# AOADMM-DataFusionFramework/Matlab-Code

Hardware: AMD Instinct MI355X
Metric: AO-ADMM outer iters/sec (+ mode-1 MTTKRP GFLOP/s), 2000^3 rank-20 CP (higher is better)
Workload: dtype f32

## Files before the change

matlab-code_amd/csrc/contract.hip:

```cpp
#include "contract.h"
#include "device_utils.h"
#include "small_dev.h"

#include <algorithm>
#include <cstdlib>

namespace aoadmm {

typedef float f32x4 __attribute__((ext_vector_type(4)));
typedef double f64x2 __attribute__((ext_vector_type(2)));
typedef double f64x4 __attribute__((ext_vector_type(4)));

static constexpr int kTileRows = 128;
static constexpr int kGroup = 8;

struct KArgs {
  const void* X;
  const void* frag;
  void* T;
  int64_t tiles_per_batch, ntiles, batch_stride, M, ld, C, Cg, trows;
  int groups_per_chunk, R;
  int flush_every;
};

// ... 661 lines not shown
  int groups_per_chunk, R;
  float inv_s;
};

template <int NT>
__global__ __launch_bounds__(256, NT <= 2 ? 2 : 1) void contract16_f16(KArgs16 a) {
  const int lane = threadIdx.x & 63;
  const int64_t wt = (int64_t)blockIdx.x * 4 + (threadIdx.x >> 6);
  if (wt >= a.ntiles) return;
  const int chunk = blockIdx.y;
  const int64_t blk = wt >> 2;
  const int m0 = (int)(wt & 3) * kTileRows;
  const int r16 = lane & 15, q = lane >> 4;
  const int64_t g0 = (int64_t)chunk * a.groups_per_chunk;
  int64_t g1 = g0 + a.groups_per_chunk;
  if (g1 > a.Cg) g1 = a.Cg;
  const int64_t ng = g1 > g0 ? g1 - g0 : 0;
  const _Float16* xp = a.X + (blk * a.Cg + g0) * kGroupHalves + (m0 + r16) * kGroup16 + 8 * q;
  const f16x8* fp = reinterpret_cast<const f16x8*>(reinterpret_cast<const char*>(a.frag) + kFragHeader16) + g0 * (NT * 128) + lane;

  f32x4 acc[NT][8];
#pragma unroll
  for (int nt = 0; nt < NT; ++nt)
#pragma unroll
    for (int t = 0; t < 8; ++t) acc[nt][t] = f32x4{0.f, 0.f, 0.f, 0.f};

  f16x8 x0[8], x1[8], x2[8];
  f16x8 f0[NT][2], f1[NT][2], f2[NT][2];
#define AO_LOAD1(XS, GI, TL) XS[TL] = __builtin_nontemporal_load(reinterpret_cast<const f16x8*>(xp + (GI) * kGroupHalves + (TL) * (16 * kGroup16)));
#define AO_LOADF(FS, GI)                                                                             \
  {                                                                                                  \
    _Pragma("unroll") for (int nt = 0; nt < NT; ++nt) {                                              \
      FS[nt][0] = fp[(GI) * (NT * 128) + nt * 128];                                                  \
      FS[nt][1] = fp[(GI) * (NT * 128) + nt * 128 + 64];                                             \
    }                                                                                                \
  }
#define AO_LOAD_STAGE(XS, FS, GI)                                                                    \
  { _Pragma("unroll") for (int tl_ = 0; tl_ < 8; ++tl_) AO_LOAD1(XS, GI, tl_) AO_LOADF(FS, GI) }
#define AO_FMA_T(XS, FS, TL)                                                                         \
  {                                                                                                  \
    _Pragma("unroll") for (int nt = 0; nt < NT; ++nt) {                                              \
      acc[nt][TL] = __builtin_amdgcn_mfma_f32_16x16x32_f16(XS[TL], FS[nt][0], acc[nt][TL], 0, 0, 0); \
      acc[nt][TL] = __builtin_amdgcn_mfma_f32_16x16x32_f16(XS[TL], FS[nt][1], acc[nt][TL], 0, 0, 0); \
    }                                                                                                \
  }
#define AO_COMPUTE_STAGE(XS, FS) { _Pragma("unroll") for (int tl_ = 0; tl_ < 8; ++tl_) AO_FMA_T(XS, FS, tl_) }
#define AO_MIX_STAGE(XC, FC, XL, FL, GI)                                                             \
  {                                                                                                  \
    _Pragma("unroll") for (int tl_ = 0; tl_ < 8; ++tl_) {                                            \
      AO_FMA_T(XC, FC, tl_) AO_LOAD1(XL, GI, tl_)                                                    \
      if (tl_ == 7) AO_LOADF(FL, GI)                                                                 \
      __builtin_amdgcn_sched_barrier(0);                                                             \
    }                                                                                                \
  }
  if (ng > 0) AO_LOAD_STAGE(x0, f0, 0)
  if (ng > 1) AO_LOAD_STAGE(x1, f1, 1)
  int64_t g = 0;
  for (; g + 5 <= ng; g += 3) {
    AO_MIX_STAGE(x0, f0, x2, f2, g + 2)
    AO_MIX_STAGE(x1, f1, x0, f0, g + 3)
    AO_MIX_STAGE(x2, f2, x1, f1, g + 4)
  }
  for (; g + 3 <= ng; g += 3) {
    if (g + 2 < ng) AO_LOAD_STAGE(x2, f2, g + 2)
    AO_COMPUTE_STAGE(x0, f0)
    if (g + 3 < ng) AO_LOAD_STAGE(x0, f0, g + 3)
    AO_COMPUTE_STAGE(x1, f1)
    if (g + 4 < ng) AO_LOAD_STAGE(x1, f1, g + 4)
    AO_COMPUTE_STAGE(x2, f2)
  }
  if (g < ng) AO_COMPUTE_STAGE(x0, f0)
  if (g + 1 < ng) AO_COMPUTE_STAGE(x1, f1)
#undef AO_LOAD1
#undef AO_LOADF
#undef AO_LOAD_STAGE
#undef AO_FMA_T
#undef AO_COMPUTE_STAGE
#undef AO_MIX_STAGE
  extern __shared__ __attribute__((aligned(16))) float t_lds[];
  float* tl = t_lds + (threadIdx.x >> 6) * (kTileRows * a.R);
  const float* tinv = reinterpret_cast<const float*>(reinterpret_cast<const char*>(a.frag) + 512);
#pragma unroll
  for (int nt = 0; nt < NT; ++nt) {
    const int r = 16 * nt + r16;
    if (r < a.R) {
      const float ti = tinv[r];
#pragma unroll
      for (int t = 0; t < 8; ++t)
#pragma unroll
        for (int i = 0; i < 4; ++i) tl[(16 * t + 4 * q + i) * a.R + r] = acc[nt][t][i] * ti * a.inv_s;
    }
  }
  {
    const int n16 = kTileRows * a.R / 4;
    f32x4* dst = reinterpret_cast<f32x4*>(a.T + ((int64_t)chunk * a.trows + blk * 512 + m0) * a.R);
    const f32x4* src = reinterpret_cast<const f32x4*>(tl);
    for (int c = lane; c < n16; c += 64) __builtin_nontemporal_store(src[c], dst + c);
  }
}

static int nt_of(int R, int prec) {
  const int w = prec == AOADMM_PREC_F32 ? 32 : 16;
  return (R + w - 1) / w;
}
static int tile_rows(int prec) { return prec == AOADMM_PREC_F64 ? kTileRows64 : kTileRows; }

size_t ContractPlan::frag_bytes(int prec) const {
  if (prec == AOADMM_PREC_F16)
    return (size_t)kFragHeader16 + (size_t)cdiv(C, kGroup16) * nt_of(R, prec) * 2048;
  const int64_t Cg = cdiv(C, kGroup);
  return (size_t)(nt_of(R, prec) * 1024 + 1152) * Cg + 8192;
}

ContractPlan make_plan(int64_t nbatch, int64_t batch_stride, int64_t M, int64_t ld, int64_t C, int R,
                       int prec) {
  ContractPlan p;
  const bool half = prec == AOADMM_PREC_F16;
  p.tprec = half ? AOADMM_PREC_F32 : prec;
  p.nbatch = nbatch; p.batch_stride = batch_stride; p.M = M; p.ld = ld; p.C = C; p.R = R;
  const int gcols = half ? kGroup16 : kGroup;
  const int64_t Cg = cdiv(C, gcols);
  const int64_t ntiles = nbatch * cdiv(M, tile_rows(prec));
  int64_t nchunk = 1;
  if (prec != AOADMM_PREC_F64) nchunk = cdiv(Cg, 2048 / gcols);
  if (ntiles < 2048) {
    int64_t want = cdiv(2048, ntiles);
    const int64_t gmin = 128 / gcols;
    int64_t maxc = Cg / gmin > 0 ? Cg / gmin : 1;
    if (want > maxc) want = maxc;
    if (want > nchunk) nchunk = want;
  }
  if (nchunk > 65535) nchunk = 65535;
  p.nchunk = (int)nchunk;
  return p;
}

ContractPlan make_lead_plan(int64_t M, int64_t ld, int64_t C, int R) {
  ContractPlan p;
  p.tprec = AOADMM_PREC_F32;
  p.nbatch = 1; p.batch_stride = 0; p.M = M; p.ld = ld; p.C = C; p.R = R;
  p.lead = true;
  const int64_t nch = cdiv(C, kLeadKC);
  p.nchunk = (int)cdiv(nch, 2048 / kLeadKC);
  return p;
}

static void launch_contract_lead(const void* X, const ContractPlan& pl, const double* F, int64_t ldF, void* frag_ws,
                                 void* T, hipStream_t s, hipEvent_t ev0, hipEvent_t ev1) {
  const int64_t Cg = cdiv(pl.C, kGroup);
  AO_REQUIRE(pl.ld % 4 == 0 && pl.ld >= 4, "f32 layout must be padded to 4");
  LArgs a;
  a.X = (const float*)X; a.frag = (const float*)frag_ws; a.T = (float*)T;
  a.M = pl.M; a.ld = pl.ld; a.C = pl.C; a.Cg = Cg; a.R = pl.R;
  a.chunks_per_slice = (int)cdiv(cdiv(pl.C, kLeadKC), pl.nchunk);
  const int64_t nblk = cdiv(pl.M, kLeadRows);
  AO_REQUIRE(nblk < (int64_t)2147483647, "tensor too large for one launch");
  dim3 grid((unsigned)nblk, (unsigned)pl.nchunk);
  const size_t sh = (size_t)2 * kLeadRows * kLeadStride * sizeof(float);
  const int nt16 = (pl.R + 15) / 16;
  const int64_t Cg16 = cdiv(pl.C, 16) + 1;
  const int64_t total = (int64_t)nt16 * Cg16 * 256;
  pack_frag_lead16_f32<<<(unsigned)cdiv(total, 256), 256, 0, s>>>(F, ldF, pl.C, pl.R, nt16, Cg16, (float*)frag_ws);
  AO_KERNEL_CHECK();
#define AO_SET(K) ensure_dynamic_lds(reinterpret_cast<const void*>(K), (int)sh);
  if (nt16 == 1) AO_SET(contract_lead16_f32<1>)
  else if (nt16 == 2) AO_SET(contract_lead16_f32<2>)
  else if (nt16 == 3) AO_SET(contract_lead16_f32<3>)
  else if (nt16 == 4) AO_SET(contract_lead16_f32<4>)
#undef AO_SET
  if (ev0) AO_HIP(hipEventRecord(ev0, s));
  if (nt16 == 1) contract_lead16_f32<1><<<grid, 256, sh, s>>>(a);
  else if (nt16 == 2) contract_lead16_f32<2><<<grid, 256, sh, s>>>(a);
  else if (nt16 == 3) contract_lead16_f32<3><<<grid, 256, sh, s>>>(a);
  else if (nt16 == 4) contract_lead16_f32<4><<<grid, 256, sh, s>>>(a);
  else throw Error(AOADMM_ERR_UNSUPPORTED, "rank > 64 not supported");
  if (ev1) AO_HIP(hipEventRecord(ev1, s));
  AO_KERNEL_CHECK();
}

static void launch_contract_half(const void* X, const ContractPlan& pl, const double* F, int64_t ldF, void* frag_ws,
                                 void* T, hipStream_t s, hipEvent_t ev0, hipEvent_t ev1) {
  AO_REQUIRE(pl.on_copy && !pl.lead && pl.M == 512 && pl.ld == 512 && pl.tprec == AOADMM_PREC_F32,
             "internal: a half operand is streamed from its pass copies only");
  const int64_t Cg = cdiv(pl.C, kGroup16);
  AO_REQUIRE(pl.batch_stride == 512 * kGroup16 * Cg && pl.nbatch > 0 && pl.C > 0, "internal: half pass copy and plan disagree");
  const int NT = nt_of(pl.R, AOADMM_PREC_F16);
  char* ws = reinterpret_cast<char*>(frag_ws);
  double* tsc = reinterpret_cast<double*>(ws);
  float* tinv = reinterpret_cast<float*>(ws + 512);
  frag16_scales_k<<<(unsigned)pl.R, 256, 0, s>>>(F, ldF, pl.C, tsc, tinv);
  AO_KERNEL_CHECK();
  pack_frag16_f16<<<(unsigned)cdiv(Cg * NT * 128, 256), 256, 0, s>>>(F, ldF, pl.C, pl.R, NT, Cg, tsc,
                                                                    reinterpret_cast<f16x8*>(ws + kFragHeader16));
  AO_KERNEL_CHECK();
  KArgs16 a;
  a.X = reinterpret_cast<const _Float16*>(X); a.frag = frag_ws; a.T = reinterpret_cast<float*>(T);
  a.ntiles = pl.nbatch * 4; a.Cg = Cg; a.trows = pl.trows();
  a.groups_per_chunk = (int)cdiv(Cg, pl.nchunk);
  a.R = pl.R;
  a.inv_s = (float)(1.0 / pl.xscale);
  AO_REQUIRE(pl.nbatch < (int64_t)2147483647, "tensor too large for one launch");
  const dim3 grid((unsigned)pl.nbatch, (unsigned)pl.nchunk);
  const size_t tsh = (size_t)4 * kTileRows * pl.R * sizeof(float);
#define AO_GO(K) { if (tsh > 65536) ensure_dynamic_lds(reinterpret_cast<const void*>(K), (int)tsh); if (ev0) AO_HIP(hipEventRecord(ev0, s)); K<<<grid, 256, tsh, s>>>(a); }
  if (NT == 1) AO_GO(contract16_f16<1>)
  else if (NT == 2) AO_GO(contract16_f16<2>)
  else if (NT == 3) AO_GO(contract16_f16<3>)
  else if (NT == 4) AO_GO(contract16_f16<4>)
  else throw Error(AOADMM_ERR_UNSUPPORTED, "rank > 64 not supported");
#undef AO_GO
  if (ev1) AO_HIP(hipEventRecord(ev1, s));
  AO_KERNEL_CHECK();
}

void launch_contract(const void* X, int prec, const ContractPlan& pl, const double* F, int64_t ldF,
                     void* frag_ws, void* T, hipStream_t s, hipEvent_t ev0, hipEvent_t ev1) {
  AO_REQUIRE(pl.R >= 1 && pl.R <= kMaxRank, "rank %d outside [1,%d]", pl.R, kMaxRank);
  if (prec == AOADMM_PREC_F16) {
    launch_contract_half(X, pl, F, ldF, frag_ws, T, s, ev0, ev1);
    return;
  }
  AO_REQUIRE(prec == AOADMM_PREC_F32 || prec == AOADMM_PREC_F64, "bad precision id %d", prec);
  AO_REQUIRE(pl.tprec == prec, "contraction plan and tensor precision disagree");
  if (pl.lead) {
    AO_REQUIRE(prec == AOADMM_PREC_F32, "leading-mode contraction exists for fp32 tensors only");
    launch_contract_lead(X, pl, F, ldF, frag_ws, T, s, ev0, ev1);
    return;
  }
  const int64_t Cg = cdiv(pl.C, kGroup);
  KArgs a;
  a.X = X; a.frag = frag_ws; a.T = T;
  a.tiles_per_batch = cdiv(pl.M, tile_rows(prec));
  a.ntiles = pl.nbatch * a.tiles_per_batch;
  a.batch_stride = pl.batch_stride; a.M = pl.M; a.ld = pl.ld; a.C = pl.C; a.Cg = Cg;
  a.trows = pl.trows();
  a.groups_per_chunk = (int)cdiv(Cg, pl.nchunk);
  a.R = pl.R;
  AO_REQUIRE(a.ntiles > 0 && pl.C > 0, "empty contraction");
  dim3 grid((unsigned)cdiv(a.ntiles, 4), (unsigned)pl.nchunk);
  AO_REQUIRE(cdiv(a.ntiles, 4) < (int64_t)2147483647, "tensor too large for one launch");
  if (prec == AOADMM_PREC_F32) {
    AO_REQUIRE(pl.ld % 4 == 0 && pl.M % 4 == 0 && pl.batch_stride % 4 == 0, "f32 layout must be padded to 4");
    const int rem = pl.R % 16;
    const bool ex = pl.R > 16 && rem >= 1 && rem <= 4;
    const int nt16 = ex ? pl.R / 16 : (pl.R + 15) / 16;
    const int64_t total = (int64_t)nt16 * Cg * 128 + (ex ? Cg * 32 : 0);
    pack_frag16_f32<<<(unsigned)cdiv(total, 256), 256, 0, s>>>(F, ldF, pl.C, pl.R, nt16, ex ? 1 : 0, Cg, (float*)frag_ws);
    AO_KERNEL_CHECK();
    size_t tsh = (size_t)4 * kTileRows * pl.R * sizeof(float);
    a.flush_every = kFlushEvery;
    if (nt16 == 1) tsh = (size_t)4 * 16384;
#define AO_GO(K) { if (tsh > 65536) ensure_dynamic_lds(reinterpret_cast<const void*>(K), (int)tsh); if (ev0) AO_HIP(hipEventRecord(ev0, s)); K<<<grid, 256, tsh, s>>>(a); }
    if (nt16 == 1 && !ex) AO_GO((contract16_f32<1, false, true>))
    else if (nt16 == 1) AO_GO((contract16_f32<1, true, true>))
    else if (nt16 == 2 && !ex) AO_GO((contract16_f32<2, false>))
    else if (nt16 == 2) AO_GO((contract16_f32<2, true>))
    else if (nt16 == 3 && !ex) AO_GO((contract16_f32<3, false>))
    else if (nt16 == 3) AO_GO((contract16_f32<3, true>))
    else if (nt16 == 4) AO_GO((contract16_f32<4, false>))
    else throw Error(AOADMM_ERR_UNSUPPORTED, "rank > 64 not supported");
#undef AO_GO
  } else {
    AO_REQUIRE(pl.ld % 2 == 0 && pl.M % 2 == 0 && pl.batch_stride % 2 == 0, "f64 layout must be padded to 2");
    const int rem = pl.R % 16;
    const bool ex = pl.R > 16 && rem >= 1 && rem <= 4;
    const int nt16 = ex ? pl.R / 16 : (pl.R + 15) / 16;
    const int64_t total = (int64_t)nt16 * Cg * 128 + (ex ? Cg * 32 : 0);
    pack_frag_f64<<<(unsigned)cdiv(total, 256), 256, 0, s>>>(F, ldF, pl.C, pl.R, nt16, ex ? 1 : 0, Cg, (double*)frag_ws);
    AO_KERNEL_CHECK();
    const size_t tsh = (size_t)4 * kTileRows64 * pl.R * sizeof(double);
#define AO_GO(K) { if (tsh > 65536) ensure_dynamic_lds(reinterpret_cast<const void*>(K), (int)tsh); if (ev0) AO_HIP(hipEventRecord(ev0, s)); K<<<grid, 256, tsh, s>>>(a); }
    if (nt16 == 1 && !ex) AO_GO((contract_f64<1, false>))
    else if (nt16 == 1) AO_GO((contract_f64<1, true>))
    else if (nt16 == 2 && !ex) AO_GO((contract_f64<2, false>))
    else if (nt16 == 2) AO_GO((contract_f64<2, true>))
    else if (nt16 == 3 && !ex) AO_GO((contract_f64<3, false>))
    else if (nt16 == 3) AO_GO((contract_f64<3, true>))
    else if (nt16 == 4) AO_GO((contract_f64<4, false>))
    else throw Error(AOADMM_ERR_UNSUPPORTED, "rank > 64 not supported");
#undef AO_GO
  }
  if (ev1) AO_HIP(hipEventRecord(ev1, s));
  AO_KERNEL_CHECK();
}

__global__ void factor_rowmajor_k(const double* __restrict__ F, int64_t ldF, int64_t rows, int R,
                                  double* __restrict__ Ft) {
  const int64_t idx = (int64_t)blockIdx.x * blockDim.x + threadIdx.x;
  if (idx >= rows * R) return;
  const int r = (int)(idx / rows);
  const int64_t a = idx - (int64_t)r * rows;
  Ft[a * R + r] = F[a + ldF * r];
}
static void factor_rowmajor(const double* F, int64_t ldF, int64_t rows, int R, double* Ft, hipStream_t s) {
  factor_rowmajor_k<<<(unsigned)cdiv(rows * R, 256), 256, 0, s>>>(F, ldF, rows, R, Ft);
  AO_KERNEL_CHECK();
}

template <typename TT, int VEC> struct TVec;
template <> struct TVec<float, 4> { typedef float type __attribute__((ext_vector_type(4))); };
template <> struct TVec<float, 1> { typedef float type; };
template <> struct TVec<double, 2> { typedef double type __attribute__((ext_vector_type(2))); };
template <> struct TVec<double, 1> { typedef double type; };
template <typename TT, int VEC>
__device__ __forceinline__ void fma_vec(double (&acc)[VEC], const TT* __restrict__ tp, const double* __restrict__ fp) {
  typedef typename TVec<TT, VEC>::type V;
  const V tv = __builtin_nontemporal_load(reinterpret_cast<const V*>(tp));
  if constexpr (VEC == 1) {
    acc[0] += (double)tv * fp[0];
  } else {
#pragma unroll
    for (int v = 0; v < VEC; ++v) acc[v] += (double)tv[v] * fp[v];
  }
}

template <typename TT, int VEC>
struct RVec {
  typename TVec<TT, VEC>::type t;
  double f[VEC];
  __device__ __forceinline__ void load(const TT* __restrict__ tp, const double* __restrict__ fp) {
    t = __builtin_nontemporal_load(reinterpret_cast<const typename TVec<TT, VEC>::type*>(tp));
#pragma unroll
    for (int v = 0; v < VEC; ++v) f[v] = fp[v];
  }
  __device__ __forceinline__ void fma(double (&acc)[VEC]) const {
    if constexpr (VEC == 1) {
      acc[0] += (double)t * f[0];
    } else {
#pragma unroll
      for (int v = 0; v < VEC; ++v) acc[v] += (double)t[v] * f[v];
    }
  }
};

template <typename TT, int VEC>
__global__ void reduce_inner_k(const TT* __restrict__ T, int nchunk, int64_t trows, int64_t A, int64_t Apad, int R,
                               const double* __restrict__ FaT, double scale, double* __restrict__ out,
                               int64_t ldOut, int rowmajor, int has_sys, SysBuild sys) {
  extern __shared__ double sh[];
  if (has_sys && blockIdx.x == 0) { sys_build_rider(sys); return; }
  const int64_t b = (int64_t)blockIdx.x - has_sys;
  const int t = threadIdx.x;
  const int64_t n = A * R, step = (int64_t)blockDim.x * VEC;
  double s0[VEC], s1[VEC], s2[VEC], s3[VEC];
#pragma unroll
  for (int v = 0; v < VEC; ++v) { s0[v] = 0; s1[v] = 0; s2[v] = 0; s3[v] = 0; }
  for (int ch = 0; ch < nchunk; ++ch) {
    const TT* Tb = T + ((int64_t)ch * trows + Apad * b) * R;
    int64_t e = (int64_t)t * VEC;
    for (; e + 3 * step < n; e += 4 * step) {
      RVec<TT, VEC> q0, q1, q2, q3;
      q0.load(Tb + e, FaT + e);
      q1.load(Tb + e + step, FaT + e + step);
      q2.load(Tb + e + 2 * step, FaT + e + 2 * step);
      q3.load(Tb + e + 3 * step, FaT + e + 3 * step);
      __builtin_amdgcn_sched_barrier(0);
      q0.fma(s0); q1.fma(s1); q2.fma(s2); q3.fma(s3);
    }
    for (; e < n; e += step) fma_vec<TT, VEC>(s0, Tb + e, FaT + e);
  }
#pragma unroll
  for (int v = 0; v < VEC; ++v) sh[t * VEC + v] = (s0[v] + s1[v]) + (s2[v] + s3[v]);
  __syncthreads();
  if (t < R) {
    const int nA = blockDim.x * VEC / R;
    double tot = 0.0;
    for (int i = 0; i < nA; ++i) tot += sh[i * R + t];
    if (rowmajor) out[b * R + t] = scale * tot;
    else out[b + ldOut * t] = scale * tot;
  }
}

template <typename TT, int VEC>
__global__ void reduce_inner2_k(const TT* __restrict__ T, int nchunk, int64_t trows, int64_t A, int64_t Apad, int64_t B,
                                int R, const double* __restrict__ FaT, double scale, double* __restrict__ out,
                                int64_t ldOut, int rowmajor, int has_sys, SysBuild sys) {
  extern __shared__ double sh[];
  if (has_sys && blockIdx.x == 0) { sys_build_rider(sys); return; }
  const int64_t b0 = 2 * ((int64_t)blockIdx.x - has_sys);
  const bool two = b0 + 1 < B;
  const int64_t b1 = two ? b0 + 1 : b0;
  const int t = threadIdx.x;
  const int64_t n = A * R, step = (int64_t)blockDim.x * VEC;
  double a0[VEC], a1[VEC], c0[VEC], c1[VEC];
#pragma unroll
  for (int v = 0; v < VEC; ++v) { a0[v] = 0; a1[v] = 0; c0[v] = 0; c1[v] = 0; }
  for (int ch = 0; ch < nchunk; ++ch) {
    const TT* Ta = T + ((int64_t)ch * trows + Apad * b0) * R;
    const TT* Tc = T + ((int64_t)ch * trows + Apad * b1) * R;
    int64_t e = (int64_t)t * VEC;
    for (; e + step < n; e += 2 * step) {
      RVec<TT, VEC> q0, q1, p0, p1;
      q0.load(Ta + e, FaT + e);
      q1.load(Ta + e + step, FaT + e + step);
      p0.t = __builtin_nontemporal_load(reinterpret_cast<const typename TVec<TT, VEC>::type*>(Tc + e));
      p1.t = __builtin_nontemporal_load(reinterpret_cast<const typename TVec<TT, VEC>::type*>(Tc + e + step));
      __builtin_amdgcn_sched_barrier(0);
#pragma unroll
      for (int v = 0; v < VEC; ++v) { p0.f[v] = q0.f[v]; p1.f[v] = q1.f[v]; }
      q0.fma(a0); q1.fma(a1); p0.fma(c0); p1.fma(c1);
    }
    for (; e < n; e += step) {
      RVec<TT, VEC> q0, p0;
      q0.load(Ta + e, FaT + e);
      p0.t = __builtin_nontemporal_load(reinterpret_cast<const typename TVec<TT, VEC>::type*>(Tc + e));
#pragma unroll
      for (int v = 0; v < VEC; ++v) p0.f[v] = q0.f[v];
      q0.fma(a0); p0.fma(c0);
    }
  }
  const int nt = blockDim.x * VEC;
#pragma unroll
  for (int v = 0; v < VEC; ++v) { sh[t * VEC + v] = a0[v] + a1[v]; sh[nt + t * VEC + v] = c0[v] + c1[v]; }
  __syncthreads();
  if (t < 2 * R) {
    const int which = t / R, r = t % R;
    if (which == 0 || two) {
      const int nA = nt / R;
      double tot = 0.0;
      for (int i = 0; i < nA; ++i) tot += sh[which * nt + i * R + r];
      const int64_t b = which ? b1 : b0;
      if (rowmajor) out[b * R + r] = scale * tot;
      else out[b + ldOut * r] = scale * tot;
    }
  }
}

size_t reduce_factor_scratch_bytes(int64_t rows, int R) { return (size_t)rows * R * sizeof(double); }

template <typename TT, int VEC>
static void launch_inner_t(const void* T, int nchunk, int64_t trows, int64_t A, int64_t Apad, int64_t B, int R,
                           const double* FaT, double scale, double* out, int64_t ldOut, hipStream_t s, int rowmajor,
                           const SysBuild* sys) {
  const int hs = sys ? 1 : 0;
  const SysBuild sb = sys ? *sys : SysBuild();
  const int rq = R / VEC;
  int threads = 256 / rq * rq;
  if (threads < rq) threads = rq;
  if (threads * VEC < R) threads = (R + VEC - 1) / VEC;
  if (B >= 1024 && 2 * R <= threads) {
    reduce_inner2_k<TT, VEC><<<(unsigned)((B + 1) / 2 + hs), threads, (size_t)2 * threads * VEC * sizeof(double), s>>>(
        (const TT*)T, nchunk, trows, A, Apad, B, R, FaT, scale, out, ldOut, rowmajor, hs, sb);
    return;
  }
  reduce_inner_k<TT, VEC><<<(unsigned)(B + hs), threads, (size_t)threads * VEC * sizeof(double), s>>>(
      (const TT*)T, nchunk, trows, A, Apad, R, FaT, scale, out, ldOut, rowmajor, hs, sb);
}

static bool sys_can_ride(const SysBuild* sys, int threads_min = 64) {
  return sys != nullptr && sys->R >= 1 && sys->R <= kSysRiderMaxR && threads_min >= 64;
}

bool launch_reduce_inner(const void* T, int tprec, int nchunk, int64_t trows, int64_t A, int64_t Apad,
                         int64_t B, int R, const double* Fa, int64_t ldFa, double scale,
                         double* out, int64_t ldOut, double* ft_scratch, hipStream_t s, const double* FaT,
                         int rowmajor_out, const SysBuild* sys) {
  AO_REQUIRE((int64_t)B < 2147483647ll, "reduce_inner: too many output rows for one launch");
  {
    const int vec = tprec == AOADMM_PREC_F32 ? (R % 4 == 0 ? 4 : 1) : (R % 2 == 0 ? 2 : 1);
    const int rq = R / vec;
    int threads = 256 / rq * rq;
    if (threads < rq) threads = rq;
    if (threads * vec < R) threads = (R + vec - 1) / vec;
    if (!sys_can_ride(sys, threads)) sys = nullptr;
  }
  if (FaT) ft_scratch = const_cast<double*>(FaT);
  else factor_rowmajor(Fa, ldFa, A, R, ft_scratch, s);
  if (tprec == AOADMM_PREC_F32) {
    if (R % 4 == 0) launch_inner_t<float, 4>(T, nchunk, trows, A, Apad, B, R, ft_scratch, scale, out, ldOut, s, rowmajor_out, sys);
    else launch_inner_t<float, 1>(T, nchunk, trows, A, Apad, B, R, ft_scratch, scale, out, ldOut, s, rowmajor_out, sys);
  } else {
    if (R % 2 == 0) launch_inner_t<double, 2>(T, nchunk, trows, A, Apad, B, R, ft_scratch, scale, out, ldOut, s, rowmajor_out, sys);
    else launch_inner_t<double, 1>(T, nchunk, trows, A, Apad, B, R, ft_scratch, scale, out, ldOut, s, rowmajor_out, sys);
  }
  AO_KERNEL_CHECK();
  return sys != nullptr;
}

static void outer_geometry(int64_t A, int64_t B, int R, int vec, int& TA, int64_t& nblkA, int& SB) {
  const int rq = (R + vec - 1) / vec;
  TA = 256 / rq;
  if (TA < 1) TA = 1;
  nblkA = cdiv(A, TA);
  int64_t sb = cdiv(2048, nblkA);
  if (sb > 64) sb = 64;
  if (sb > B) sb = B;
  if (sb < 1) sb = 1;
  SB = (int)sb;
}
static int outer_vec(int tprec, int R) {
  if (tprec == AOADMM_PREC_F32) return R % 4 == 0 ? 4 : 1;
  return R % 2 == 0 ? 2 : 1;
}

size_t reduce_outer_scratch_bytes(int64_t A, int64_t B, int R) {
  size_t worst = 0;
  for (int vec : {1, 2, 4}) {
    int TA, SB; int64_t nb;
    outer_geometry(A, B, R, vec, TA, nb, SB);
    worst = std::max(worst, (size_t)SB * A * R * sizeof(double));
  }
  return worst;
}

template <typename TT, int VEC>
__global__ void reduce_outer_k(const TT* __restrict__ T, int nchunk, int64_t trows, int64_t A,
                               int64_t Apad, int64_t B, int R, int TA, const double* __restrict__ FbT,
                               double* __restrict__ part, int has_sys, SysBuild sys) {
  if (has_sys && blockIdx.x == 0) {
    if (blockIdx.y == 0) sys_build_rider(sys);
    return;
  }
  const int t = threadIdx.x;
  const int rq = R / VEC;
  const int al = t / rq, r = (t - al * rq) * VEC;
  const int64_t a = ((int64_t)blockIdx.x - has_sys) * TA + al;
  const int SB = gridDim.y, sb = blockIdx.y;
  const int64_t bper = (B + SB - 1) / SB;
  const int64_t b0 = sb * bper;
  int64_t b1 = b0 + bper;
  if (b1 > B) b1 = B;
  if (al >= TA || a >= A) return;
  const int64_t bs = Apad * R;
  double s0[VEC], s1[VEC], s2[VEC], s3[VEC];
#pragma unroll
  for (int v = 0; v < VEC; ++v) { s0[v] = 0; s1[v] = 0; s2[v] = 0; s3[v] = 0; }
  for (int ch = 0; ch < nchunk; ++ch) {
    const TT* Tc = T + (int64_t)ch * trows * R + a * R + r;
    const double* Fr = FbT + r;
    int64_t b = b0;
    for (; b + 3 < b1; b += 4) {
      RVec<TT, VEC> q0, q1, q2, q3;
      q0.load(Tc + bs * b, Fr + b * R);
      q1.load(Tc + bs * (b + 1), Fr + (b + 1) * R);
      q2.load(Tc + bs * (b + 2), Fr + (b + 2) * R);
      q3.load(Tc + bs * (b + 3), Fr + (b + 3) * R);
      __builtin_amdgcn_sched_barrier(0);
      q0.fma(s0); q1.fma(s1); q2.fma(s2); q3.fma(s3);
    }
    for (; b < b1; ++b) fma_vec<TT, VEC>(s0, Tc + bs * b, Fr + b * R);
  }
#pragma unroll
  for (int v = 0; v < VEC; ++v) part[((int64_t)sb * A + a) * R + r + v] = (s0[v] + s1[v]) + (s2[v] + s3[v]);
}

__global__ void reduce_outer_fin(const double* __restrict__ part, int SB, int64_t A, int R, double scale,
                                 double* __restrict__ out, int64_t ldOut, int rowmajor) {
  int64_t idx = (int64_t)blockIdx.x * blockDim.x + threadIdx.x;
  if (idx >= A * R) return;
  const int64_t a = idx / R;
  const int r = (int)(idx - a * R);
  double t0 = 0.0, t1 = 0.0;
  int s = 0;
  const int64_t ar = A * R;
  for (; s + 7 < SB; s += 8) {
    const double v0 = part[(int64_t)s * ar + idx], v1 = part[(int64_t)(s + 1) * ar + idx];
    const double v2 = part[(int64_t)(s + 2) * ar + idx], v3 = part[(int64_t)(s + 3) * ar + idx];
    const double v4 = part[(int64_t)(s + 4) * ar + idx], v5 = part[(int64_t)(s + 5) * ar + idx];
    const double v6 = part[(int64_t)(s + 6) * ar + idx], v7 = part[(int64_t)(s + 7) * ar + idx];
    t0 += v0; t1 += v1; t0 += v2; t1 += v3; t0 += v4; t1 += v5; t0 += v6; t1 += v7;
  }
  for (; s + 1 < SB; s += 2) {
    t0 += part[(int64_t)s * ar + idx];
    t1 += part[(int64_t)(s + 1) * ar + idx];
  }
  if (s < SB) t0 += part[(int64_t)s * ar + idx];
  if (rowmajor) out[idx] = scale * (t0 + t1);
  else out[a + ldOut * r] = scale * (t0 + t1);
}

template <typename TT, int VEC>
static void launch_outer_t(const void* T, int nchunk, int64_t trows, int64_t A, int64_t Apad, int64_t B, int R,
                           const double* FbT, double* scratch, int& SB, hipStream_t s, const SysBuild* sys) {
  int TA; int64_t nb;
  outer_geometry(A, B, R, VEC, TA, nb, SB);
  int threads = TA * (R / VEC);
  threads = (threads + 63) / 64 * 64;
  const int hs = sys ? 1 : 0;
  reduce_outer_k<TT, VEC><<<dim3((unsigned)(nb + hs), (unsigned)SB), threads, 0, s>>>((const TT*)T, nchunk, trows, A, Apad, B,
                                                                                    R, TA, FbT, scratch, hs, sys ? *sys : SysBuild());
}

bool launch_reduce_outer(const void* T, int tprec, int nchunk, int64_t trows, int64_t A, int64_t Apad,
                         int64_t B, int R, const double* Fb, int64_t ldFb, double scale,
                         double* out, int64_t ldOut, double* scratch, double* ft_scratch, hipStream_t s,
                         const double* FbT, int rowmajor_out, const SysBuild* sys) {
  if (!sys_can_ride(sys)) sys = nullptr;
  if (FbT) ft_scratch = const_cast<double*>(FbT);
  else factor_rowmajor(Fb, ldFb, B, R, ft_scratch, s);
  int SB = 1;
  const int vec = outer_vec(tprec, R);
  if (tprec == AOADMM_PREC_F32) {
    if (vec == 4) launch_outer_t<float, 4>(T, nchunk, trows, A, Apad, B, R, ft_scratch, scratch, SB, s, sys);
    else launch_outer_t<float, 1>(T, nchunk, trows, A, Apad, B, R, ft_scratch, scratch, SB, s, sys);
  } else {
    if (vec == 2) launch_outer_t<double, 2>(T, nchunk, trows, A, Apad, B, R, ft_scratch, scratch, SB, s, sys);
    else launch_outer_t<double, 1>(T, nchunk, trows, A, Apad, B, R, ft_scratch, scratch, SB, s, sys);
  }
  AO_KERNEL_CHECK();
  reduce_outer_fin<<<(unsigned)cdiv(A * R, 256), 256, 0, s>>>(scratch, SB, A, R, scale, out, ldOut, rowmajor_out);
  AO_KERNEL_CHECK();
  return sys != nullptr;
}

template <typename TT, int RMAX>
__global__ __launch_bounds__(256) void small_mttkrp_k(SmallMttkrp a, int has_sys, SysBuild sys) {
  extern __shared__ double sf[];
  if (has_sys && blockIdx.x == 0) { sys_build_rider(sys); return; }
  const int row = (int)blockIdx.x - has_sys;
  const int R = a.R, Na = a.Na, Nb = a.Nb;
  double* fa = sf;
  double* fb = sf + (size_t)Na * R;
  double* red = fb + (size_t)(Nb > 0 ? Nb : 1) * R;
  for (int e = threadIdx.x; e < Na * R; e += 256) { const int i = e / R, r = e - i * R; fa[e] = a.Fa[i + a.lda * r]; }
  for (int e = threadIdx.x; e < Nb * R; e += 256) { const int i = e / R, r = e - i * R; fb[e] = a.Fb ? a.Fb[i + a.ldb * r] : 1.0; }
  __syncthreads();
  const TT* X = reinterpret_cast<const TT*>(a.X) + (int64_t)row * a.sn;
  double acc[RMAX];
#pragma unroll
  for (int r = 0; r < RMAX; ++r) acc[r] = 0.0;
  const int npairs = Na * Nb;
  for (int p = threadIdx.x; p < npairs; p += 256) {
    const int ia = p % Na, ib = p / Na;
    const double x = (double)X[(int64_t)ia * a.sa + (int64_t)ib * a.sb];
#pragma unroll
    for (int r = 0; r < RMAX; ++r)
      if (r < R) acc[r] += x * (fa[ia * R + r] * fb[ib * R + r]);
  }
  const int lane = threadIdx.x & 63, w = threadIdx.x >> 6;
#pragma unroll
  for (int r = 0; r < RMAX; ++r) {
    const double v = wave_sum(acc[r]);
    if (lane == 0) red[w * RMAX + r] = v;
  }
  __syncthreads();
  if ((int)threadIdx.x < R) {
    const int r = threadIdx.x;
    const double tot = (red[r] + red[RMAX + r]) + (red[2 * RMAX + r] + red[3 * RMAX + r]);
    a.out[row + a.ldOut * r] = a.scale * tot;
  }
}

bool small_mttkrp_ok(int64_t elems, int nd, const int64_t* dims, int R) {
  const bool off = getenv("AOADMM_NO_SMALL_MTTKRP") != nullptr;
  if (off || elems > kSmallMttkrpElems || !(nd == 2 || nd == 3) || R > 16) return false;
  int64_t sum = 0;
  for (int i = 0; i < nd; ++i) sum += dims[i];
  return (size_t)(sum * R + 64) * sizeof(double) <= 40 * 1024;
}

bool small_mttkrp(const SmallMttkrp& a, int prec, int64_t rows, hipStream_t s, const SysBuild* sys) {
  if (!sys_can_ride(sys)) sys = nullptr;
  const int hs = sys ? 1 : 0;
  const SysBuild sb = sys ? *sys : SysBuild();
  AO_REQUIRE(a.R >= 1 && a.R <= 16 && rows >= 1 && a.Na >= 1 && a.Nb >= 1, "small_mttkrp: bad sizes");
  const int rmax = a.R <= 4 ? 4 : (a.R <= 8 ? 8 : 16);
  const size_t lds = ((size_t)(a.Na + a.Nb) * a.R + 4 * rmax) * sizeof(double);
  AO_REQUIRE(lds <= 48 * 1024, "small_mttkrp: factors do not fit LDS");
#define AO_SM(TT, RM) small_mttkrp_k<TT, RM><<<(unsigned)(rows + hs), 256, lds, s>>>(a, hs, sb)
  if (prec == AOADMM_PREC_F32) { if (rmax == 4) AO_SM(float, 4); else if (rmax == 8) AO_SM(float, 8); else AO_SM(float, 16); }
  else { if (rmax == 4) AO_SM(double, 4); else if (rmax == 8) AO_SM(double, 8); else AO_SM(double, 16); }
#undef AO_SM
  AO_KERNEL_CHECK();
  return sys != nullptr;
}

template <typename TT>
__global__ void t_to_colmajor_k(const TT* __restrict__ T, int nchunk, int64_t trows, int64_t A, int R,
                                double scale, double* __restrict__ out, int64_t ldOut) {
  int64_t idx = (int64_t)blockIdx.x * blockDim.x + threadIdx.x;
  if (idx >= A * R) return;
  const int64_t a = idx / R;
  const int r = (int)(idx - a * R);
  double tot = 0.0;
  for (int ch = 0; ch < nchunk; ++ch) tot += (double)T[(int64_t)ch * trows * R + idx];
  out[a + ldOut * r] = scale * tot;
}

void launch_t_to_colmajor(const void* T, int tprec, int nchunk, int64_t trows, int64_t A, int R, double scale,
                          double* out, int64_t ldOut, hipStream_t s) {
  const unsigned nb = (unsigned)cdiv(A * R, 256);
  if (tprec == AOADMM_PREC_F32) t_to_colmajor_k<float><<<nb, 256, 0, s>>>((const float*)T, nchunk, trows, A, R, scale, out, ldOut);
  else t_to_colmajor_k<double><<<nb, 256, 0, s>>>((const double*)T, nchunk, trows, A, R, scale, out, ldOut);
  AO_KERNEL_CHECK();
}

}
```

Before: 129.5.

## Restructure inner/outer MTTKRP reductions with multi-slab blocking and deeper load batching

Rewrites the inner reduction so each block handles S=1/2/4 output slabs (4 when B>=2000). The shared factor loads are reused across slabs, and 8 loads per thread are in flight instead of 4. The outer reduction now sweeps contiguous spans of A*R with two vectors per thread and 8 B-rows unrolled. Its slice count is derived from a bytes-in-flight target rather than a fixed block count. Thread counts come from a cache-line-aligned heuristic. This raises register pressure and changes the reduction order, and the scratch sizing now assumes f32 element size.

Result: no change. 129.0 (-0.4%).

```diff
diff --git a/matlab-code_amd/csrc/contract.hip b/matlab-code_amd/csrc/contract.hip
--- a/matlab-code_amd/csrc/contract.hip
+++ b/matlab-code_amd/csrc/contract.hip
@@ -987,127 +987,104 @@
 template <> struct TVec<float, 1> { typedef float type; };
 template <> struct TVec<double, 2> { typedef double type __attribute__((ext_vector_type(2))); };
 template <> struct TVec<double, 1> { typedef double type; };
+static constexpr int kInnerLoads = 8;
+static constexpr int kOuterVecs = 2;
+static constexpr int kOuterRows = 8;
+static constexpr int64_t kOuterBytesInFlight = (int64_t)12 << 20;
+
 template <typename TT, int VEC>
-__device__ __forceinline__ void fma_vec(double (&acc)[VEC], const TT* __restrict__ tp, const double* __restrict__ fp) {
+__device__ __forceinline__ typename TVec<TT, VEC>::type load_t(const TT* __restrict__ p) {
+  return __builtin_nontemporal_load(reinterpret_cast<const typename TVec<TT, VEC>::type*>(p));
+}
+template <typename V, int VEC>
+__device__ __forceinline__ double lane_of(const V& x, int v) {
+  if constexpr (VEC == 1) return (double)x;
+  else return (double)x[v];
+}
+
+static int sweep_threads(int R, int vec, int tsize) {
+  const int rq = R / vec;
+  const int line = 128 / (vec * tsize);
+  int a = rq, b = line;
+  while (b) { const int c = a % b; a = b; b = c; }
+  int unit = rq / a * line;
+  if (unit > 256) unit = rq;
+  return unit >= 256 ? unit : 256 / unit * unit;
+}
+static int sweep_vec(int tprec, int R) {
+  if (tprec == AOADMM_PREC_F32) return R % 4 == 0 ? 4 : 1;
+  return R % 2 == 0 ? 2 : 1;
+}
+
+template <typename TT, int VEC, int S>
+__global__ __launch_bounds__(256, S == 1 ? 3 : 4) void reduce_inner_k(const TT* __restrict__ T, int nchunk, int64_t trows, int64_t A,
+                                                      int64_t Apad, int64_t B, int R, const double* __restrict__ FaT,
+                                                      double scale, double* __restrict__ out, int64_t ldOut,
+                                                      int rowmajor, int has_sys, SysBuild sys) {
+  constexpr int E = kInnerLoads / S;
   typedef typename TVec<TT, VEC>::type V;
-  const V tv = __builtin_nontemporal_load(reinterpret_cast<const V*>(tp));
-  if constexpr (VEC == 1) {
-    acc[0] += (double)tv * fp[0];
-  } else {
-#pragma unroll
-    for (int v = 0; v < VEC; ++v) acc[v] += (double)tv[v] * fp[v];
-  }
-}
-
-template <typename TT, int VEC>
-struct RVec {
-  typename TVec<TT, VEC>::type t;
-  double f[VEC];
-  __device__ __forceinline__ void load(const TT* __restrict__ tp, const double* __restrict__ fp) {
-    t = __builtin_nontemporal_load(reinterpret_cast<const typename TVec<TT, VEC>::type*>(tp));
-#pragma unroll
-    for (int v = 0; v < VEC; ++v) f[v] = fp[v];
-  }
-  __device__ __forceinline__ void fma(double (&acc)[VEC]) const {
-    if constexpr (VEC == 1) {
-      acc[0] += (double)t * f[0];
-    } else {
-#pragma unroll
-      for (int v = 0; v < VEC; ++v) acc[v] += (double)t[v] * f[v];
-    }
-  }
-};
-
-template <typename TT, int VEC>
-__global__ void reduce_inner_k(const TT* __restrict__ T, int nchunk, int64_t trows, int64_t A, int64_t Apad, int R,
-                               const double* __restrict__ FaT, double scale, double* __restrict__ out,
-                               int64_t ldOut, int rowmajor, int has_sys, SysBuild sys) {
   extern __shared__ double sh[];
   if (has_sys && blockIdx.x == 0) { sys_build_rider(sys); return; }
-  const int64_t b = (int64_t)blockIdx.x - has_sys;
+  const int64_t g = (int64_t)blockIdx.x - has_sys;
   const int t = threadIdx.x;
   const int64_t n = A * R, step = (int64_t)blockDim.x * VEC;
-  double s0[VEC], s1[VEC], s2[VEC], s3[VEC];
-#pragma unroll
-  for (int v = 0; v < VEC; ++v) { s0[v] = 0; s1[v] = 0; s2[v] = 0; s3[v] = 0; }
+  int64_t slab[S];
+#pragma unroll
+  for (int s = 0; s < S; ++s) slab[s] = (g * S + s < B ? g * S + s : B - 1) * Apad * R;
+  double acc[S][2][VEC];
+#pragma unroll
+  for (int s = 0; s < S; ++s)
+#pragma unroll
+    for (int v = 0; v < VEC; ++v) { acc[s][0][v] = 0; acc[s][1][v] = 0; }
   for (int ch = 0; ch < nchunk; ++ch) {
-    const TT* Tb = T + ((int64_t)ch * trows + Apad * b) * R;
+    const TT* Tc = T + (int64_t)ch * trows * R;
     int64_t e = (int64_t)t * VEC;
-    for (; e + 3 * step < n; e += 4 * step) {
-      RVec<TT, VEC> q0, q1, q2, q3;
-      q0.load(Tb + e, FaT + e);
-      q1.load(Tb + e + step, FaT + e + step);
-      q2.load(Tb + e + 2 * step, FaT + e + 2 * step);
-      q3.load(Tb + e + 3 * step, FaT + e + 3 * step);
+    for (; e + (E - 1) * step < n; e += E * step) {
+      V tv[S][E];
+      double f[E][VEC];
+#pragma unroll
+      for (int i = 0; i < E; ++i) {
+#pragma unroll
+        for (int s = 0; s < S; ++s) tv[s][i] = load_t<TT, VEC>(Tc + slab[s] + e + i * step);
+#pragma unroll
+        for (int v = 0; v < VEC; ++v) f[i][v] = FaT[e + i * step + v];
+      }
       __builtin_amdgcn_sched_barrier(0);
-      q0.fma(s0); q1.fma(s1); q2.fma(s2); q3.fma(s3);
-    }
-    for (; e < n; e += step) fma_vec<TT, VEC>(s0, Tb + e, FaT + e);
-  }
-#pragma unroll
-  for (int v = 0; v < VEC; ++v) sh[t * VEC + v] = (s0[v] + s1[v]) + (s2[v] + s3[v]);
+#pragma unroll
+      for (int i = 0; i < E; ++i)
+#pragma unroll
+        for (int s = 0; s < S; ++s)
+#pragma unroll
+          for (int v = 0; v < VEC; ++v) acc[s][i & 1][v] += lane_of<V, VEC>(tv[s][i], v) * f[i][v];
+    }
+    for (; e < n; e += step) {
+      V tv[S];
+      double f[VEC];
+#pragma unroll
+      for (int s = 0; s < S; ++s) tv[s] = load_t<TT, VEC>(Tc + slab[s] + e);
+#pragma unroll
+      for (int v = 0; v < VEC; ++v) f[v] = FaT[e + v];
+#pragma unroll
+      for (int s = 0; s < S; ++s)
+#pragma unroll
+        for (int v = 0; v < VEC; ++v) acc[s][0][v] += lane_of<V, VEC>(tv[s], v) * f[v];
+    }
+  }
+  const int nt = blockDim.x * VEC;
+#pragma unroll
+  for (int s = 0; s < S; ++s)
+#pragma unroll
+    for (int v = 0; v < VEC; ++v) sh[s * nt + t * VEC + v] = acc[s][0][v] + acc[s][1][v];
   __syncthreads();
-  if (t < R) {
-    const int nA = blockDim.x * VEC / R;
+  for (int q = t; q < S * R; q += blockDim.x) {
+    const int s = q / R, r = q - s * R;
+    const int64_t b = g * S + s;
+    if (b >= B) continue;
+    const int nA = nt / R;
     double tot = 0.0;
-    for (int i = 0; i < nA; ++i) tot += sh[i * R + t];
-    if (rowmajor) out[b * R + t] = scale * tot;
-    else out[b + ldOut * t] = scale * tot;
-  }
-}
-
-template <typename TT, int VEC>
-__global__ void reduce_inner2_k(const TT* __restrict__ T, int nchunk, int64_t trows, int64_t A, int64_t Apad, int64_t B,
-                                int R, const double* __restrict__ FaT, double scale, double* __restrict__ out,
-                                int64_t ldOut, int rowmajor, int has_sys, SysBuild sys) {
-  extern __shared__ double sh[];
-  if (has_sys && blockIdx.x == 0) { sys_build_rider(sys); return; }
-  const int64_t b0 = 2 * ((int64_t)blockIdx.x - has_sys);
-  const bool two = b0 + 1 < B;
-  const int64_t b1 = two ? b0 + 1 : b0;
-  const int t = threadIdx.x;
-  const int64_t n = A * R, step = (int64_t)blockDim.x * VEC;
-  double a0[VEC], a1[VEC], c0[VEC], c1[VEC];
-#pragma unroll
-  for (int v = 0; v < VEC; ++v) { a0[v] = 0; a1[v] = 0; c0[v] = 0; c1[v] = 0; }
-  for (int ch = 0; ch < nchunk; ++ch) {
-    const TT* Ta = T + ((int64_t)ch * trows + Apad * b0) * R;
-    const TT* Tc = T + ((int64_t)ch * trows + Apad * b1) * R;
-    int64_t e = (int64_t)t * VEC;
-    for (; e + step < n; e += 2 * step) {
-      RVec<TT, VEC> q0, q1, p0, p1;
-      q0.load(Ta + e, FaT + e);
-      q1.load(Ta + e + step, FaT + e + step);
-      p0.t = __builtin_nontemporal_load(reinterpret_cast<const typename TVec<TT, VEC>::type*>(Tc + e));
-      p1.t = __builtin_nontemporal_load(reinterpret_cast<const typename TVec<TT, VEC>::type*>(Tc + e + step));
-      __builtin_amdgcn_sched_barrier(0);
-#pragma unroll
-      for (int v = 0; v < VEC; ++v) { p0.f[v] = q0.f[v]; p1.f[v] = q1.f[v]; }
-      q0.fma(a0); q1.fma(a1); p0.fma(c0); p1.fma(c1);
-    }
-    for (; e < n; e += step) {
-      RVec<TT, VEC> q0, p0;
-      q0.load(Ta + e, FaT + e);
-      p0.t = __builtin_nontemporal_load(reinterpret_cast<const typename TVec<TT, VEC>::type*>(Tc + e));
-#pragma unroll
-      for (int v = 0; v < VEC; ++v) p0.f[v] = q0.f[v];
-      q0.fma(a0); p0.fma(c0);
-    }
-  }
-  const int nt = blockDim.x * VEC;
-#pragma unroll
-  for (int v = 0; v < VEC; ++v) { sh[t * VEC + v] = a0[v] + a1[v]; sh[nt + t * VEC + v] = c0[v] + c1[v]; }
-  __syncthreads();
-  if (t < 2 * R) {
-    const int which = t / R, r = t % R;
-    if (which == 0 || two) {
-      const int nA = nt / R;
-      double tot = 0.0;
-      for (int i = 0; i < nA; ++i) tot += sh[which * nt + i * R + r];
-      const int64_t b = which ? b1 : b0;
-      if (rowmajor) out[b * R + r] = scale * tot;
-      else out[b + ldOut * r] = scale * tot;
-    }
+    for (int i = 0; i < nA; ++i) tot += sh[s * nt + i * R + r];
+    if (rowmajor) out[b * R + r] = scale * tot;
+    else out[b + ldOut * r] = scale * tot;
   }
 }
 
@@ -1119,21 +1096,24 @@
                            const SysBuild* sys) {
   const int hs = sys ? 1 : 0;
   const SysBuild sb = sys ? *sys : SysBuild();
-  const int rq = R / VEC;
-  int threads = 256 / rq * rq;
-  if (threads < rq) threads = rq;
-  if (threads * VEC < R) threads = (R + VEC - 1) / VEC;
-  if (B >= 1024 && 2 * R <= threads) {
-    reduce_inner2_k<TT, VEC><<<(unsigned)((B + 1) / 2 + hs), threads, (size_t)2 * threads * VEC * sizeof(double), s>>>(
+  const int threads = sweep_threads(R, VEC, (int)sizeof(TT));
+  const size_t lds = (size_t)threads * VEC * sizeof(double);
+  if (B >= 2000) {
+    reduce_inner_k<TT, VEC, 4><<<(unsigned)((B + 3) / 4 + hs), threads, 4 * lds, s>>>(
         (const TT*)T, nchunk, trows, A, Apad, B, R, FaT, scale, out, ldOut, rowmajor, hs, sb);
     return;
   }
-  reduce_inner_k<TT, VEC><<<(unsigned)(B + hs), threads, (size_t)threads * VEC * sizeof(double), s>>>(
-      (const TT*)T, nchunk, trows, A, Apad, R, FaT, scale, out, ldOut, rowmajor, hs, sb);
-}
-
-static bool sys_can_ride(const SysBuild* sys, int threads_min = 64) {
-  return sys != nullptr && sys->R >= 1 && sys->R <= kSysRiderMaxR && threads_min >= 64;
+  if (B >= 1024) {
+    reduce_inner_k<TT, VEC, 2><<<(unsigned)((B + 1) / 2 + hs), threads, 2 * lds, s>>>(
+        (const TT*)T, nchunk, trows, A, Apad, B, R, FaT, scale, out, ldOut, rowmajor, hs, sb);
+    return;
+  }
+  reduce_inner_k<TT, VEC, 1><<<(unsigned)(B + hs), threads, lds, s>>>(
+      (const TT*)T, nchunk, trows, A, Apad, B, R, FaT, scale, out, ldOut, rowmajor, hs, sb);
+}
+
+static bool sys_can_ride(const SysBuild* sys) {
+  return sys != nullptr && sys->R >= 1 && sys->R <= kSysRiderMaxR;
 }
 
 bool launch_reduce_inner(const void* T, int tprec, int nchunk, int64_t trows, int64_t A, int64_t Apad,
@@ -1141,14 +1121,8 @@
                          double* out, int64_t ldOut, double* ft_scratch, hipStream_t s, const double* FaT,
                          int rowmajor_out, const SysBuild* sys) {
   AO_REQUIRE((int64_t)B < 2147483647ll, "reduce_inner: too many output rows for one launch");
-  {
-    const int vec = tprec == AOADMM_PREC_F32 ? (R % 4 == 0 ? 4 : 1) : (R % 2 == 0 ? 2 : 1);
-    const int rq = R / vec;
-    int threads = 256 / rq * rq;
-    if (threads < rq) threads = rq;
-    if (threads * vec < R) threads = (R + vec - 1) / vec;
-    if (!sys_can_ride(sys, threads)) sys = nullptr;
-  }
+  AO_REQUIRE(R >= 1 && R <= 64 && B >= 1, "reduce_inner: bad sizes");
+  if (!sys_can_ride(sys)) sys = nullptr;
   if (FaT) ft_scratch = const_cast<double*>(FaT);
   else factor_rowmajor(Fa, ldFa, A, R, ft_scratch, s);
   if (tprec == AOADMM_PREC_F32) {
@@ -1162,71 +1136,86 @@
   return sys != nullptr;
 }
 
-static void outer_geometry(int64_t A, int64_t B, int R, int vec, int& TA, int64_t& nblkA, int& SB) {
-  const int rq = (R + vec - 1) / vec;
-  TA = 256 / rq;
-  if (TA < 1) TA = 1;
-  nblkA = cdiv(A, TA);
-  int64_t sb = cdiv(2048, nblkA);
+static int outer_slices(int64_t A, int64_t B, int R, int tsize) {
+  int64_t sb = cdiv(kOuterBytesInFlight, (int64_t)kOuterRows * A * R * tsize);
   if (sb > 64) sb = 64;
-  if (sb > B) sb = B;
+  if (sb > B / kOuterRows) sb = B / kOuterRows;
   if (sb < 1) sb = 1;
-  SB = (int)sb;
-}
-static int outer_vec(int tprec, int R) {
-  if (tprec == AOADMM_PREC_F32) return R % 4 == 0 ? 4 : 1;
-  return R % 2 == 0 ? 2 : 1;
+  return (int)sb;
 }
 
 size_t reduce_outer_scratch_bytes(int64_t A, int64_t B, int R) {
-  size_t worst = 0;
-  for (int vec : {1, 2, 4}) {
-    int TA, SB; int64_t nb;
-    outer_geometry(A, B, R, vec, TA, nb, SB);
-    worst = std::max(worst, (size_t)SB * A * R * sizeof(double));
-  }
-  return worst;
+  return (size_t)outer_slices(A, B, R, (int)sizeof(float)) * A * R * sizeof(double);
 }
 
 template <typename TT, int VEC>
-__global__ void reduce_outer_k(const TT* __restrict__ T, int nchunk, int64_t trows, int64_t A,
-                               int64_t Apad, int64_t B, int R, int TA, const double* __restrict__ FbT,
-                               double* __restrict__ part, int has_sys, SysBuild sys) {
+__global__ __launch_bounds__(256) void reduce_outer_k(const TT* __restrict__ T, int nchunk, int64_t trows, int64_t n,
+                                                      int64_t bs, int64_t B, int R, const double* __restrict__ FbT,
+                                                      double* __restrict__ part, int has_sys, SysBuild sys) {
+  constexpr int K = kOuterVecs, U = kOuterRows;
+  typedef typename TVec<TT, VEC>::type V;
   if (has_sys && blockIdx.x == 0) {
     if (blockIdx.y == 0) sys_build_rider(sys);
     return;
   }
-  const int t = threadIdx.x;
-  const int rq = R / VEC;
-  const int al = t / rq, r = (t - al * rq) * VEC;
-  const int64_t a = ((int64_t)blockIdx.x - has_sys) * TA + al;
+  const int64_t step = (int64_t)blockDim.x * VEC;
+  const int64_t e0 = ((int64_t)blockIdx.x - has_sys) * K * step + (int64_t)threadIdx.x * VEC;
+  if (e0 >= n) return;
+  const int r = (int)(e0 % R);
+  int64_t off[K];
+#pragma unroll
+  for (int j = 0; j < K; ++j) off[j] = e0 + j * step < n ? j * step : 0;
   const int SB = gridDim.y, sb = blockIdx.y;
   const int64_t bper = (B + SB - 1) / SB;
   const int64_t b0 = sb * bper;
   int64_t b1 = b0 + bper;
   if (b1 > B) b1 = B;
-  if (al >= TA || a >= A) return;
-  const int64_t bs = Apad * R;
-  double s0[VEC], s1[VEC], s2[VEC], s3[VEC];
-#pragma unroll
-  for (int v = 0; v < VEC; ++v) { s0[v] = 0; s1[v] = 0; s2[v] = 0; s3[v] = 0; }
+  double acc[K][VEC];
+#pragma unroll
+  for (int j = 0; j < K; ++j)
+#pragma unroll
+    for (int v = 0; v < VEC; ++v) acc[j][v] = 0;
   for (int ch = 0; ch < nchunk; ++ch) {
-    const TT* Tc = T + (int64_t)ch * trows * R + a * R + r;
+    const TT* Tc = T + (int64_t)ch * trows * R + e0;
     const double* Fr = FbT + r;
     int64_t b = b0;
-    for (; b + 3 < b1; b += 4) {
-      RVec<TT, VEC> q0, q1, q2, q3;
-      q0.load(Tc + bs * b, Fr + b * R);
-      q1.load(Tc + bs * (b + 1), Fr + (b + 1) * R);
-      q2.load(Tc + bs * (b + 2), Fr + (b + 2) * R);
-      q3.load(Tc + bs * (b + 3), Fr + (b + 3) * R);
+    for (; b + U <= b1; b += U) {
+      V tv[U][K];
+      double f[U][VEC];
+#pragma unroll
+      for (int u = 0; u < U; ++u) {
+#pragma unroll
+        for (int j = 0; j < K; ++j) tv[u][j] = load_t<TT, VEC>(Tc + bs * (b + u) + off[j]);
+#pragma unroll
+        for (int v = 0; v < VEC; ++v) f[u][v] = Fr[(b + u) * R + v];
+      }
       __builtin_amdgcn_sched_barrier(0);
-      q0.fma(s0); q1.fma(s1); q2.fma(s2); q3.fma(s3);
-    }
-    for (; b < b1; ++b) fma_vec<TT, VEC>(s0, Tc + bs * b, Fr + b * R);
-  }
-#pragma unroll
-  for (int v = 0; v < VEC; ++v) part[((int64_t)sb * A + a) * R + r + v] = (s0[v] + s1[v]) + (s2[v] + s3[v]);
+#pragma unroll
+      for (int u = 0; u < U; ++u)
+#pragma unroll
+        for (int j = 0; j < K; ++j)
+#pragma unroll
+          for (int v = 0; v < VEC; ++v) acc[j][v] += lane_of<V, VEC>(tv[u][j], v) * f[u][v];
+    }
+    for (; b < b1; ++b) {
+      V tv[K];
+      double f[VEC];
+#pragma unroll
+      for (int j = 0; j < K; ++j) tv[j] = load_t<TT, VEC>(Tc + bs * b + off[j]);
+#pragma unroll
+      for (int v = 0; v < VEC; ++v) f[v] = Fr[b * R + v];
+#pragma unroll
+      for (int j = 0; j < K; ++j)
+#pragma unroll
+        for (int v = 0; v < VEC; ++v) acc[j][v] += lane_of<V, VEC>(tv[j], v) * f[v];
+    }
+  }
+#pragma unroll
+  for (int j = 0; j < K; ++j) {
+    if (e0 + j * step >= n) break;
+#pragma unroll
+    for (int v = 0; v < VEC; ++v) part[(int64_t)sb * n + e0 + j * step + v] = acc[j][v];
+  }
 }
 
 __global__ void reduce_outer_fin(const double* __restrict__ part, int SB, int64_t A, int R, double scale,
@@ -1256,25 +1245,25 @@
 
 template <typename TT, int VEC>
 static void launch_outer_t(const void* T, int nchunk, int64_t trows, int64_t A, int64_t Apad, int64_t B, int R,
-                           const double* FbT, double* scratch, int& SB, hipStream_t s, const SysBuild* sys) {
-  int TA; int64_t nb;
-  outer_geometry(A, B, R, VEC, TA, nb, SB);
-  int threads = TA * (R / VEC);
-  threads = (threads + 63) / 64 * 64;
+                           const double* FbT, double* scratch, int SB, hipStream_t s, const SysBuild* sys) {
+  const int threads = sweep_threads(R, VEC, (int)sizeof(TT));
+  const int64_t spans = cdiv(A * R, (int64_t)threads * VEC * kOuterVecs);
+  AO_REQUIRE(spans < 2147483647ll, "reduce_outer: too many output rows for one launch");
   const int hs = sys ? 1 : 0;
-  reduce_outer_k<TT, VEC><<<dim3((unsigned)(nb + hs), (unsigned)SB), threads, 0, s>>>((const TT*)T, nchunk, trows, A, Apad, B,
-                                                                                    R, TA, FbT, scratch, hs, sys ? *sys : SysBuild());
+  reduce_outer_k<TT, VEC><<<dim3((unsigned)(spans + hs), (unsigned)SB), threads, 0, s>>>(
+      (const TT*)T, nchunk, trows, A * R, Apad * R, B, R, FbT, scratch, hs, sys ? *sys : SysBuild());
 }
 
 bool launch_reduce_outer(const void* T, int tprec, int nchunk, int64_t trows, int64_t A, int64_t Apad,
                          int64_t B, int R, const double* Fb, int64_t ldFb, double scale,
                          double* out, int64_t ldOut, double* scratch, double* ft_scratch, hipStream_t s,
                          const double* FbT, int rowmajor_out, const SysBuild* sys) {
+  AO_REQUIRE(R >= 1 && R <= 64 && A >= 1 && B >= 1, "reduce_outer: bad sizes");
   if (!sys_can_ride(sys)) sys = nullptr;
   if (FbT) ft_scratch = const_cast<double*>(FbT);
   else factor_rowmajor(Fb, ldFb, B, R, ft_scratch, s);
-  int SB = 1;
-  const int vec = outer_vec(tprec, R);
+  const int vec = sweep_vec(tprec, R);
+  const int SB = outer_slices(A, B, R, tprec == AOADMM_PREC_F32 ? (int)sizeof(float) : (int)sizeof(double));
   if (tprec == AOADMM_PREC_F32) {
     if (vec == 4) launch_outer_t<float, 4>(T, nchunk, trows, A, Apad, B, R, ft_scratch, scratch, SB, s, sys);
     else launch_outer_t<float, 1>(T, nchunk, trows, A, Apad, B, R, ft_scratch, scratch, SB, s, sys);
```
